# adelacvg/detail_tts

Hardware: AMD Instinct MI355X
Metric: generated audio seconds/sec (24 kHz), 10 s prompt, batch 8 per GPU (higher is better)
Workload: dtype f32; 1 GPU; configs[2]: 1xMI355X batch-8, 10 s prompts (T_ref=936), 234 codes -> 9.984 s audio per utterance; GPT KV-cache decode + 50-step CFG diffusion + flow-VAE/HiFiGAN vocoder, seed-0 random-init weights; batch_per_gpu=8, codes=234, diffusion_steps=50, parallelism=replica x1

## Files before the change

### detail_tts_amd/csrc/model.h

```cpp
#pragma once
#include <map>
#include <memory>
#include <atomic>
#include <thread>
#include <cstring>
#include <memory>
#include <mutex>
#include <string>
#include <unordered_map>
#include <vector>

#include "attention.h"
#include "attn_probs.h"
#include "common.h"
#include "conv_gemm.h"
#include "conv_x3.h"
#include "diff_loss.h"
#include "diff_schedule.h"
#include "disc.h"
#include "flowvae_fwd.h"
#include "gpt_kernels.h"
#include "ops.h"
#include "uncond_cache.h"
#include "../../include/detail_hip.h"

namespace dtts {

struct PackedConv {
    const float* w = nullptr;
    const float* b = nullptr;
    int Cin = 0, CinP = 0, Cout = 0, CoutP = 0, KW = 1;
    const void* w3 = nullptr;
};

static inline int packed_cout(int cout) { return cout > 64 ? round_up(cout, 128) : (cout > 32 ? 64 : 32); }

static inline int gn_groups(int C) {
    int groups = 32;
    while (C % groups) groups /= 2;
    return groups;
}

struct AttnBlockW {
    const float *gn_g = nullptr, *gn_b = nullptr, *bias_tab = nullptr;
    PackedConv qkv, proj;
    int C = 0, H = 0;
};

struct ResBlockW {
    const float *gn1_g = nullptr, *gn1_b = nullptr, *gn2_g = nullptr, *gn2_b = nullptr;
    PackedConv c1, c2, emb;
    int index = 0;
};

struct DiffLayerW {
    ResBlockW rb;
    AttnBlockW at;
};

struct MelStyleW {
    PackedConv sp0, sp1, t0, t1, qkv, afc, fc;
    int n_mel = 0, hidden = 0, out = 0;
};

struct EncLayerW {
    PackedConv qkv, o, f1, f2;
    const float *ek = nullptr, *ev = nullptr, *g1 = nullptr, *b1 = nullptr, *g2 = nullptr, *b2 = nullptr;
};

struct WnW {
    PackedConv cond;
    std::vector<PackedConv> in, res, skip;
    int n_layers = 0;
};

struct CouplingW {
    PackedConv pre, post;
    WnW enc;
};

struct PosteriorW {
    PackedConv pre, proj;
    WnW enc;
    int spec_channels = 0;
};

struct DiscPeriodW {
    const float *w0 = nullptr, *b0 = nullptr;
    PackedConv c[4], post;
};

struct DiscW {
    const float *sw[5] = {nullptr, nullptr, nullptr, nullptr, nullptr}, *sb[5] = {nullptr, nullptr, nullptr, nullptr, nullptr};
    PackedConv s5, s_post;
    DiscPeriodW per[5];
};

struct DiscLayout {
    long long off[DISC_MAPS + 1];
// ... 220 lines not shown
    void op_resblock1(int stage, int branch, const float* x, const int* lens_host, int B, int T, float* y, hipStream_t s);
    void op_wn(int flow, const float* h, const float* g, const int* lens_host, int B, int T, float* out, hipStream_t s);
    void posterior_encode(const float* spec, int spec_ch, const int* lens_host, const float* g, int B, int T, const float* noise, unsigned long long seed,
                          const int* sample_ids_host, float* z, float* m_q, float* logs_q, hipStream_t s);
    void flow_forward(const float* z, const float* g, const int* lens_host, int B, int T, float* z_p, hipStream_t s);
    void slice_segments(const float* x, const int* ids_host, int B, int C, int T, int seg, float* out, hipStream_t s);
    void kl_loss(const float* z_p, const float* logs_q, const float* m_p, const float* logs_p, const int* lens_host, int B, int C, int T,
                 float* out, hipStream_t s);
    void flowvae_forward(const float* mel, const float* spec, int spec_ch, const int* lens_host, int B, int T, const float* noise, unsigned long long seed,
                         const int* sample_ids_host, const int* ids_slice_host, int seg, float* o, float* z, float* z_p, float* m_p,
                         float* logs_p, float* m_q, float* logs_q, float* quantized, hipStream_t s);
    void bind_discriminator(const void* blob, size_t nbytes, const char* const* names, const unsigned long long* offsets,
                            const unsigned long long* numels, int n, hipStream_t stream);
    void disc_forward(const float* y, const float* y_hat, int B, int t, float* maps, hipStream_t s);
    void disc_losses(int n_maps, const float* const* r, const float* const* g, const long long* map_numel, int n_scores,
                     const float* const* dr, const float* const* dg, const long long* score_numel, float* out, hipStream_t s);
    void spec_to_mel(const float* spec, int B, int spec_ch, int T, float* mel_out, hipStream_t s);
    void op_conv1d_grouped(const float* x, const float* w, const float* bias, int B, int Cin, int Tin, int Cout, int groups, int K, int stride,
                           int pad, float slope, float* y, hipStream_t s);
    void op_period_split(const float* wav, int B, int t, int p, float* out, hipStream_t s);
    void flowvae_stage_losses(const float* mel, const float* spec, int spec_ch, const int* lens_host, int B, int T, const float* noise,
                              unsigned long long seed, const int* sample_ids_host, const int* ids_slice_host, int seg, const float* wav, int L,
                              float* o, float* z, float* z_p, float* m_p, float* logs_p, float* m_q, float* logs_q, float* quantized,
                              float* work, float* losses, hipStream_t s);
    void op_enc_p(const float* mel, const int* lens_host, int B, int T, float* m_p, float* logs_p, hipStream_t s);
    void enc_p_fwd(const float* mel, const int* dl, int B, int T, float* x, float* y, float* qkv, float* att, float* ffn, float* relk, float* ml,
                   float* stats, hipStream_t s, bool padded_batch = false);
    void vq_decode(const int* codes_host, const int* ncodes_host, int nmax, const float* refer, const int* refer_lens_host, int Tr,
                   int B, float* mel_out, hipStream_t s, const float* g_in = nullptr);
    void resample(const float* x, int B, int L, const float* kernel, int orig, int neu, int width, float* y, int Lout, hipStream_t s);
    void mel_spectrogram(const float* wav, const int* lens_host, int B, int L, int n_fft, int hop, float* mel_out, int Tmax, hipStream_t s,
                         float* spec_out = nullptr);
    void vq_encode(const float* mel, const int* lens_host, int B, int T, int* codes_out, float* xvq_out, hipStream_t s);
    void op_attention_block(const char* prefix, const float* x, const int* lens_host, int B, int C, int T, float* y, hipStream_t s);
    void op_resblock(const char* prefix, const float* x, const int* lens_host, int B, int T, int step, float* y, hipStream_t s);
    void op_conv1d(const char* name, const float* x, const int* lens_in_host, int B, int Cin, int Tin, int Cout, int KW, int stride,
                   int dil, int pad, int pro_act, int epi_act, int gate, int phases, const float* res, float* y, int Tout_alloc,
                   hipStream_t s);
    void op_conv1d_x3(const char* name, const float* x, const int* lens_host, int B, int Cin, int T, int Cout, int KW, int epi_act,
                      float out_scale, int gate, const float* badd, const float* res, int p1, int ksplit_max, float* y, ConvX3Launch* chosen,
                      hipStream_t s);
    void op_attention_x3(const char* name, const float* x, const int* lens_host, int B, int Cin, int T, int H, const float* bias_tab, int p1,
                         int out_f32, void* y, void* img_out, ConvX3Launch* conv_chosen, AttnX3Launch* attn_chosen, hipStream_t s);
    void op_attention(const float* qkv, const int* lens_host, int B, int rows, int cs, int T, int H, int D, int q_off, int k_off, int v_off,
                      int head_stride, float scale, const float* bias_tab, int causal, const float* band, int band_w, float* y, float* ml,
                      hipStream_t s);
    void op_attention_rel(const float* qkv, const int* lens_host, int B, int T, int H, int D, const float* ek, const float* ev, int W,
                          float scale, float* y, float* relk, float* ml, hipStream_t s);
    void op_philox_normal(float* out, int n, int B, unsigned long long seed, const int* sample_ids_host, int stage, int step,
                          hipStream_t s);

    void set_option(const std::string& key, int value) {
        if (key == "two_streams") opt_two_streams_ = value != 0;
        else if (key == "conv_x3") {
            DTTS_REQUIRE(value != 0 || !opt_trunk_fp16_, "conv_x3 = 0 (exact fp32 kernels) has no trunk_fp16 mode: set trunk_fp16 = 0 first");
            opt_conv_x3_ = value != 0;
        }
        else if (key == "trunk_fp16") {
            DTTS_REQUIRE(value == 0 || value == 1, "trunk_fp16: 0 or 1");
            DTTS_REQUIRE(value == 0 || use_x3(), "trunk_fp16 = 1 needs the split-precision kernels (conv_x3 = 1): the exact fp32 kernels have no one-product mode");
            opt_trunk_fp16_ = value != 0;
        }
        else if (key == "gpt_graph") opt_gpt_graph_ = value != 0;
        else if (key == "x3_range_check") opt_range_check_ = value != 0;
        else if (key == "gpt_token_kernel") { opt_gpt_token_ = value != 0; if (value != 0) tok_failed_ = false; gpt_drop_graphs(); }
        else if (key == "gpt_fuse_proj") { DTTS_REQUIRE(value == 0 || value == 1, "gpt_fuse_proj: 0 or 1"); opt_gpt_fuse_proj_ = value != 0; gpt_drop_graphs(); }
        else if (key == "gpt_token_exclusive_cu") { opt_tok_exclusive_ = value != 0; gpt_drop_graphs(); }
        else if (key == "gpt_token_min_rows") { DTTS_REQUIRE(value == 1 || value == 4 || value == 8, "gpt_token_min_rows: 1, 4 or 8"); opt_tok_min_rows_ = value; gpt_drop_graphs(); }
        else if (key == "gpt_token_wgs") { DTTS_REQUIRE(value == 128 || value == 64 || value == 32, "gpt_token_wgs: 128, 64 or 32"); opt_tok_wgs_ = value; gpt_drop_graphs(); }
        else if (key == "gpt_token_fault") opt_tok_fault_ = value;
        else if (key == "gpt_token_fault_eos") opt_tok_fault_eos_ = value;
        else if (key == "gpt_prompt_raw") opt_prompt_raw_ = value != 0;
        else if (key == "gpt_beam_skip_reorder") { opt_beam_skip_reorder_ = value != 0; gpt_drop_graphs(); }
        else if (key == "cfg_streams") opt_cfg_streams_ = value < 0 ? 0 : value;
        else if (key == "conv_cols") opt_conv_cols_ = value != 0;
        else if (key == "uncond_cache_mb") set_uncond_cache_mb(value);
        else if (key == "voc_chain_planes") opt_voc_chain_ = value != 0;
        else if (key == "voc_x3") opt_voc_x3_ = value != 0;
        else if (key == "x3_fault") opt_x3_fault_ = value;
        else if (key == "attn_ksplit_cus") set_attn_ksplit_cus(value);
        else if (key == "attn_ksplit") set_attn_ksplit(value);
        else if (key == "ln_reg") set_ln_channels_reg(value != 0);
        else if (key == "conv_small_tiles") set_conv_small_tiles(value);
        else if (key == "conv_stages") set_conv_stages(value);
        else throw Error(-1, "unknown option '" + key + "'");
    }
    int get_option(const std::string& key) const {
        if (key == "conv_x3") return use_x3() ? 1 : 0;
        if (key == "trunk_fp16") return opt_trunk_fp16_ ? 1 : 0;
        if (key == "gpt_fuse_proj") return opt_gpt_fuse_proj_ ? 1 : 0;
        throw Error(-1, "option '" + key + "' cannot be read back");
    }
    std::string last_error;
    dtts_config cfg;
    int device;

private:
    friend struct Stage;
    const float* W(const std::string& name, size_t numel) const;
    const float* Wopt(const std::string& name, size_t numel) const;
    PackedConv conv(const std::string& name, int Cin, int Cout, int KW, bool bias = true, int cout_p = 0) const;
    AttnBlockW attn_block(const std::string& prefix, int C, int H) const;
    ResBlockW res_block(const std::string& prefix, int C, int index) const;
    void resblock1_fwd(const ResBlock1W& rb, const float* x, float* tmp, float* out, int ch, const int* lens, int B, int T, hipStream_t s,
                       void* xs = nullptr);
    bool vocoder_x3() const;
    void wn_fwd(const WnW& c, float* h, const float* g, int gin, float* Gc, float* acts, float* h2, float* skip, const int* dl, int B,
                int T, hipStream_t s);
    WnW wn_w(const std::string& prefix, int n_layers) const;
    void enc_q_fwd(const float* spec, int spec_ch, const float* g, const int* dl, int B, int T, float* stats, hipStream_t s);
    void flow_fwd(const float* z, const float* g, const int* dl, int B, int T, float* z_p, hipStream_t s);
    size_t enc_q_ws_bytes(int B, int T) const;
    size_t flow_ws_bytes(int B, int T) const;
    std::vector<int> stage_lens(const int* lens_host, int B, int T, const char* who) const;
    void build_diffusion(hipStream_t s);
    void build_vocoder(hipStream_t s);
    void build_gpt(hipStream_t s);
    void gpt_head_and_sample(hipStream_t s);
    struct GptForced {
        float* enc = nullptr;
        int L = 0;
        std::vector<int> tl, ml;
    };
    struct GptAttnRequest {
        int mode = 0;
        const int* layers = nullptr;
        int n_layers = 0;
        const float* w = nullptr;
        float* out = nullptr;
        int nq_max = 0, nk_max = 0;
    };
    struct GptAttnCapture {
        GptAttnRequest req;
        const int *q0 = nullptr, *nq = nullptr, *k0 = nullptr, *nk = nullptr;
        const float* w = nullptr;
    };
    GptForced gpt_teacher_forced(const float* refer, const int* refer_lens_host, int Tr, const int* text_host, const int* text_lens_host,
                                 int Lt_max, const int* codes_host, const int* ncodes_host, int n_max, int B, size_t extra_ws_bytes,
                                 hipStream_t s, const float* cond_in = nullptr, const GptAttnRequest* attn = nullptr);
    void score_head(const PackedConv& head, const float* lat, long long lat_bs, int lat_cs, const int* targets_host, const int* ntargets_host,
                    int n_max, int B, float* logprob_out, float* logits_out, hipStream_t s);
    void gpt_step_launches(hipStream_t s);
    hipGraphExec_t gpt_capture(int n);
    void gpt_drop_graphs();
    void build_vq();
    void build_frontend();
    void gpt_prefill_layers(float* x, const int* lens, int B, int L, float* kv_cache, long long kv_layer_stride, long long kv_bs,
                            int kv_cs, hipStream_t s, const GptAttnCapture* capture = nullptr);
    void gpt_capture_probs(const GptAttnCapture& c, int layer, const float* qkv, const int* lens, int B, int L, hipStream_t s);
    MelStyleW mel_style_w(const std::string& prefix, int n_mel, int hidden, int out) const;
    ConvParams cp(const float* x, int cin, float* y, int cout, int B, int T, int Ta, const int* lens) const;
    ConvParams cp(const float* x, int cin, int Tin, int Tin_a, const int* len_in, float* y, int cout, int Nout, int Nout_a, const int* len_out,
                  int B) const;
    static void with_planes(ConvParams& p, const void* xs, int T) { p.x3 = xs; p.x3_tp = x3_tp(T); }
    static void with_res(ConvParams& p, const float* res, long long bs, int cs) { p.res = res; p.res_bs = bs; p.res_cs = cs; }

    const int* upload_ints(const int* host, int n, hipStream_t s);
    void register_cols(const int* lens_dev, const int* lens_host, int nb, int T, hipStream_t s);

    void run_conv(const PackedConv& pc, ConvParams p, hipStream_t s, ConvX3Launch* chosen = nullptr) const;
    struct TrunkIo {
        const int* lens;
        int B, T, Ta;
        hipStream_t s;
        float* ab;
        void* xs = nullptr;
        bool p1 = false;
// ... 231 lines not shown
```

### detail_tts_amd/csrc/model.hip

```cpp
#include "model.h"
#include <algorithm>
#include <cmath>
#include <cstring>

namespace dtts {

static thread_local Arena* t_arena_override = nullptr;
Arena* arena_override() { return t_arena_override; }
ArenaUse::ArenaUse(Arena& a) : prev_(t_arena_override) { t_arena_override = &a; }
ArenaUse::~ArenaUse() { t_arena_override = prev_; }

static thread_local bool t_row_invariant = false;
RowInvariantLaunches::RowInvariantLaunches() : prev_(t_row_invariant) { t_row_invariant = true; }
RowInvariantLaunches::~RowInvariantLaunches() { t_row_invariant = prev_; }
bool RowInvariantLaunches::on() { return t_row_invariant; }

Arena::~Arena() {
    if (base_) (void)hipFree(base_);
}

void Arena::ensure(size_t bytes) {
    if (bytes > cap_) {
        DTTS_CHECK_HIP(hipDeviceSynchronize());
        if (base_) DTTS_CHECK_HIP(hipFree(base_));
// ... 200 lines not shown
    r.gn1_b = W(p + ".in_layers.0.bias", C);
    r.c1 = conv(p + ".in_layers.2", C, C, 1);
    r.emb = conv(p + ".emb_layers.1", C, 2 * C, 1);
    r.gn2_g = W(p + ".out_layers.0.weight", C);
    r.gn2_b = W(p + ".out_layers.0.bias", C);
    r.c2 = conv(p + ".out_layers.3", C, C, 3);
    return r;
}

void Model::bind_weights(const void* blob, size_t nbytes, const char* const* names, const unsigned long long* offsets,
                         const unsigned long long* numels, int n, hipStream_t stream) {
    weights_.clear();
    bound_ = false;
    {
        std::lock_guard<std::mutex> lk(ucache_mu_);
        ++bind_gen_;
        ucache_.invalidate_all();
    }
    for (int i = 0; i < n; ++i) {
        DTTS_REQUIRE((offsets[i] + numels[i]) * sizeof(float) <= nbytes, "weight table entry outside the blob");
        DTTS_REQUIRE(offsets[i] % 4 == 0, "weight offsets must be 16-byte aligned");
        weights_[names[i]] = {static_cast<const float*>(blob) + offsets[i], (size_t)numels[i]};
    }
    if (weights_.count("diffusion.inp_block.wp")) build_diffusion(stream);
    has_vocoder_ = weights_.count("dec.conv_pre.wp") != 0;
    if (has_vocoder_) build_vocoder(stream);
    has_gpt_ = weights_.count("gpt.mel_head.wp") != 0;
    if (has_gpt_) build_gpt(stream);
    has_vq_ = weights_.count("quantizer.table") != 0;
    if (has_vq_) build_vq();
    has_frontend_ = weights_.count("frontend.dft.wp") != 0;
    if (has_frontend_) build_frontend();
    bound_ = true;
}

ConvParams Model::cp(const float* x, int cin, float* y, int cout, int B, int T, int Ta, const int* lens) const {
    return cp(x, cin, T, Ta, lens, y, cout, T, Ta, lens, B);
}

ConvParams Model::cp(const float* x, int cin, int Tin, int Tin_a, const int* len_in, float* y, int cout, int Nout, int Nout_a,
                     const int* len_out, int B) const {
    ConvParams p;
    p.B = B;
    p.Tin = Tin;
    p.Nout = Nout;
    p.len_in = len_in;
    p.len_out = len_out;
    p.x = x;
    p.x_bs = (long long)cin * Tin_a;
    p.x_cs = Tin_a;
    p.y = y;
    p.y_bs = (long long)cout * Nout_a;
    p.y_cs = Nout_a;
    return p;
}

static void attach_cols(ConvParams& p) {
    if (t_col_tables.empty() || !p.len_out || p.len_out != p.len_in || p.Nout != p.Tin || p.stride != 1 || p.phases != 1) return;
    for (const ColTable& e : t_col_tables)
        if (p.len_out >= e.lens && p.len_out + p.B <= e.lens + e.nb && p.Nout == e.T) {
            const int b0 = (int)(p.len_out - e.lens), c0 = e.prefix[b0], c1 = e.prefix[b0 + p.B];
            if (c1 > c0 && c1 - c0 < p.B * cdiv(p.Nout, X3_BN)) {
                p.cols = e.cols + c0;
                p.ncols = c1 - c0;
                p.cols_b0 = b0;
            }
            return;
        }
}

void Model::run_conv(const PackedConv& pc, ConvParams p, hipStream_t s, ConvX3Launch* chosen) const {
    p.w = pc.w;
    if (!p.bias) p.bias = pc.b;
    p.Cin = pc.Cin;
    p.CinP = pc.CinP;
    p.Cout = pc.Cout;
    p.CoutP = pc.CoutP;
    p.KW = pc.KW;
    if (p.x3) {
        DTTS_REQUIRE(pc.w3, "conv has no split-precision weights");
        p.w3 = pc.w3;
        attach_cols(p);
        if (RowInvariantLaunches::on()) p.ksplit_max = 1;
        launch_conv_x3(p, s, chosen);
        return;
    }
    launch_conv_gemm(p, s);
}

void Model::op_conv1d(const char* name, const float* x, const int* lens_in_host, int B, int Cin, int Tin, int Cout, int KW,
                      int stride, int dil, int pad, int pro_act, int epi_act, int gate, int phases, const float* res, float* y,
                      int Tout_alloc, hipStream_t s) {
    DTTS_REQUIRE(!weights_.empty(), "weights not bound");
    const int rows = Cout * (phases > 1 ? phases : 1);
    PackedConv pc = conv(name, Cin, rows, KW, Wopt(std::string(name) + ".bp", (size_t)packed_cout(rows)) != nullptr);
    const int Nout = (Tin + 2 * pad - dil * (KW - 1) - 1) / stride + 1;
    std::vector<int> li(B), lo(B);
    for (int b = 0; b < B; ++b) {
        li[b] = lens_in_host ? lens_in_host[b] : Tin;
        lo[b] = (li[b] + 2 * pad - dil * (KW - 1) - 1) / stride + 1;
    }
    const int* dli = upload_ints(li.data(), B, s);
    const int* dlo = upload_ints(lo.data(), B, s);
    const int cout_real = gate ? Cout / 2 : Cout;
    ConvParams p = cp(x, Cin, Tin, Tin, dli, y, cout_real, Nout, Tout_alloc, dlo, B);
    p.stride = stride;
    p.dil = dil;
    p.pad = pad;
    p.pro_act = pro_act;
    p.pro_slope = 0.1f;
    p.epi_act = epi_act;
    p.epi_slope = 0.1f;
    p.gate = gate;
    p.phases = phases > 1 ? phases : 1;
    if (res) with_res(p, res, p.y_bs, Tout_alloc);
    run_conv(pc, p, s);
}

void Model::op_conv1d_x3(const char* name, const float* x, const int* lens_host, int B, int Cin, int T, int Cout, int KW, int epi_act,
                         float out_scale, int gate, const float* badd, const float* res, int p1, int ksplit_max, float* y,
                         ConvX3Launch* chosen, hipStream_t s) {
    DTTS_REQUIRE(!weights_.empty(), "weights not bound");
    DTTS_REQUIRE(name && x && y, "op_conv1d_x3: null argument");
    DTTS_REQUIRE(B > 0 && B <= 65535 && T > 0 && T <= (1 << 20) && Cin > 0 && Cin <= (1 << 16) && Cout > 0 && Cout <= (1 << 16), "op_conv1d_x3: sizes");
    DTTS_REQUIRE(KW == 1 || KW == 3, "op_conv1d_x3: k = 1 or k = 3 (same padding) only");
    DTTS_REQUIRE(Cin % 16 == 0, "op_conv1d_x3: input channels must be a multiple of 16 (one K-step; the split passes write 8-channel chunks)");
    const int CoutP = packed_cout(Cout);
    DTTS_REQUIRE(CoutP % 128 == 0, "op_conv1d_x3: packed output rows must be a multiple of the 128-row tile (Cout > 64)");
    DTTS_REQUIRE(p1 == 0 || p1 == 1, "op_conv1d_x3: p1 is 0 or 1");
    DTTS_REQUIRE(gate == GATE_NONE || gate == GATE_TANH_SIGMOID, "op_conv1d_x3: gate is none or tanh * sigmoid");
    DTTS_REQUIRE(!p1 || (Cin % 32 == 0 && gate == GATE_NONE), "op_conv1d_x3 one-product mode: input channels a multiple of 32, no gate");
    DTTS_REQUIRE(epi_act == ACT_NONE || epi_act == ACT_SILU || epi_act == ACT_LRELU || epi_act == ACT_TANH, "op_conv1d_x3: epilogue activation");
    DTTS_REQUIRE(ksplit_max >= 0, "op_conv1d_x3: ksplit_max");
    const bool rows16 = (reinterpret_cast<unsigned long long>(y) & 15ull) == 0 && T % 4 == 0;
    if (gate != GATE_NONE) {
        DTTS_REQUIRE(KW == 1 && !res && epi_act == ACT_NONE && out_scale == 1.f && Cout % 2 == 0,
                     "op_conv1d_x3 gated epilogue: 1x1 conv, no residual / activation / scale, an even number of rows");
        DTTS_REQUIRE(rows16, "op_conv1d_x3 gated epilogue: rows of y must be 16-byte aligned (T a multiple of 4)");
    } else {
        DTTS_REQUIRE(!badd, "op_conv1d_x3: badd only with the gate");
    }
    const int nt = cdiv(T, X3_BN);
    DTTS_REQUIRE((long long)(CoutP / 128) * nt * B <= (1 << 22), "op_conv1d_x3: launch too large");
    std::vector<int> l(B);
    for (int b = 0; b < B; ++b) {
        l[b] = lens_host ? lens_host[b] : T;
        DTTS_REQUIRE(l[b] >= 0 && l[b] <= T, "op_conv1d_x3: lengths must lie in [0, T]");
    }
    PackedConv pc = conv(name, Cin, Cout, KW, Wopt(std::string(name) + ".bp", (size_t)CoutP) != nullptr);
    DTTS_REQUIRE(pc.CinP == Cin && pc.CoutP == CoutP, "op_conv1d_x3: packed weight shape");
    const size_t w3_bytes = (size_t)KW * (Cin / 8) * 2 * CoutP * 16;
    ws().ensure(w3_bytes + x3_bytes(B, Cin, T) + 8192);
    void* w3 = ws().raw(w3_bytes);
    void* xs = ws().raw(x3_bytes(B, Cin, T));
    launch_split_weights(pc.w, KW, pc.CinP, pc.CoutP, w3, s);
    pc.w3 = w3;
    const int* dl = upload_ints(l.data(), B, s);
    const long long x_bs = (long long)Cin * T;
    launch_split_planes(x, x_bs, T, nullptr, ACT_NONE, dl, T, B, Cin, xs, s);
    register_cols(dl, l.data(), B, T, s);
    ConvParams p = cp(x, Cin, y, gate != GATE_NONE ? Cout / 2 : Cout, B, T, T, dl);
    p.pad = KW == 3 ? 1 : 0;
    p.epi_act = epi_act;
    p.epi_slope = 0.1f;
    p.out_scale = out_scale;
    p.gate = gate;
// ... 176 lines not shown
```

Baseline: 180.5 audio_s/s.

## Add 16x16x32 MFMA variant of split-precision conv kernel and dispatch to it

Adds a new conv_x3s kernel that computes the split-precision (fp16 planes) conv GEMM with mfma_f32_16x16x32_f16 instead of the 32x32x16 shape. It uses hand-scheduled LDS reads with exec-masked half-wave loads, multi-stage global_load_lds pipelining, and optional k-split reduction. The new kernel is selected by default for eligible convs (k=1 or k=3, no gate/activation epilogue), with fallback to the old kernel otherwise. The aim is higher MFMA throughput and better LDS-read overlap in the vocoder and diffusion convs. In exchange it adds a large, complex inline-asm kernel that could carry correctness or register-pressure risk.

```diff
diff --git a/detail_tts_amd/csrc/conv_x3s.h b/detail_tts_amd/csrc/conv_x3s.h
--- /dev/null
+++ b/detail_tts_amd/csrc/conv_x3s.h
@@ -0,0 +1,12 @@
+#pragma once
+#include "conv_x3.h"
+
+namespace dtts {
+
+constexpr int CONV_X3_SHAPE_DEFAULT = 1;
+void set_conv_x3_shape(int v);
+int conv_x3_shape();
+void set_conv_x3s_stages(int n);
+bool launch_conv_x3s(const ConvParams& p, hipStream_t s, ConvX3Launch* chosen = nullptr);
+
+}
diff --git a/detail_tts_amd/csrc/conv_x3s.hip b/detail_tts_amd/csrc/conv_x3s.hip
--- /dev/null
+++ b/detail_tts_amd/csrc/conv_x3s.hip
@@ -0,0 +1,483 @@
+#include <algorithm>
+#include <atomic>
+#include <cstdio>
+#include <cstdlib>
+#include <type_traits>
+#include <utility>
+
+#include "conv_x3s.h"
+#include "prof.h"
+#include "split3.h"
+
+namespace dtts {
+
+typedef float f32x4 __attribute__((ext_vector_type(4)));
+
+namespace {
+constexpr int NPL = XS_PLANES, NK = 2 * NPL;
+constexpr int BM = 128, BN = X3_BN;
+constexpr int WTILE = NK * BM * 16;
+constexpr int XMAIN = NK * BN * 16;
+constexpr int XBUF = XMAIN + NK * 2 * 16;
+
+template <int OFF> __device__ __forceinline__ void rd(hf8& dst, unsigned addr) { asm volatile("ds_read_b128 %0, %1 offset:%2" : "=v"(dst) : "v"(addr), "n"(OFF)); }
+template <int OFF> __device__ __forceinline__ void rd_lo4(hf8 (&a)[4], unsigned wa) {
+    asm volatile("s_mov_b32 exec_hi, 0\n\t"
+                 "ds_read_b128 %0, %4 offset:%5\n\tds_read_b128 %1, %4 offset:%6\n\tds_read_b128 %2, %4 offset:%7\n\tds_read_b128 %3, %4 offset:%8\n\t"
+                 "s_mov_b64 exec, -1"
+                 : "+v"(a[0]), "+v"(a[1]), "+v"(a[2]), "+v"(a[3]) : "v"(wa), "n"(OFF), "n"(OFF + 256), "n"(OFF + 512), "n"(OFF + 768));
+}
+template <int XOFS, int WOFS> __device__ __forceinline__ void rd_hi10(hf8 (&b)[6], hf8 (&a)[4], unsigned xa, unsigned x5, unsigned wa) {
+    asm volatile("s_mov_b32 exec_lo, 0\n\t"
+                 "ds_read_b128 %0, %10 offset:%13\n\tds_read_b128 %1, %10 offset:%14\n\tds_read_b128 %2, %10 offset:%15\n\tds_read_b128 %3, %10 offset:%16\n\t"
+                 "ds_read_b128 %4, %10 offset:%17\n\tds_read_b128 %5, %11 offset:%13\n\t"
+                 "ds_read_b128 %6, %12 offset:%18\n\tds_read_b128 %7, %12 offset:%19\n\tds_read_b128 %8, %12 offset:%20\n\tds_read_b128 %9, %12 offset:%21\n\t"
+                 "s_mov_b64 exec, -1"
+                 : "+v"(b[0]), "+v"(b[1]), "+v"(b[2]), "+v"(b[3]), "+v"(b[4]), "+v"(b[5]), "+v"(a[0]), "+v"(a[1]), "+v"(a[2]), "+v"(a[3])
+                 : "v"(xa), "v"(x5), "v"(wa), "n"(XOFS), "n"(XOFS + 256), "n"(XOFS + 512), "n"(XOFS + 768), "n"(XOFS + 1024), "n"(WOFS), "n"(WOFS + 256),
+                   "n"(WOFS + 512), "n"(WOFS + 768));
+}
+template <class T> struct ic_value { static constexpr int value = 0; };
+template <int V> struct ic_value<std::integral_constant<int, V>> { static constexpr int value = V; };
+template <int N> __device__ __forceinline__ void wait1(hf8& a) { asm volatile("s_waitcnt lgkmcnt(%1)" : "+v"(a) : "n"(N)); }
+template <int N> __device__ __forceinline__ void wait7(hf8 (&b)[6], hf8& a) {
+    asm volatile("s_waitcnt lgkmcnt(%7)" : "+v"(b[0]), "+v"(b[1]), "+v"(b[2]), "+v"(b[3]), "+v"(b[4]), "+v"(b[5]), "+v"(a) : "n"(N));
+}
+
+template <int... K, class F>
+__device__ __forceinline__ void for_each_step(std::integer_sequence<int, K...>, F&& f) {
+    (f(std::integral_constant<int, K>{}), ...);
+}
+
+template <bool KW3, int NSTG>
+__global__ __launch_bounds__(256, 2) void conv_x3s_kernel(ConvParams p) {
+    constexpr int KW = KW3 ? 3 : 1, D = NSTG - 1;
+    constexpr int CB = 2;
+    auto chunk_of = [](int kind) { return (kind & 1) * NPL + (kind >> 1); };
+    constexpr int XOFF = NSTG * WTILE;
+    extern __shared__ __attribute__((aligned(16))) unsigned char smem[];
+    const int tid = threadIdx.x, lane = tid & 63, wave = __builtin_amdgcn_readfirstlane(tid >> 6);
+    const int l15 = lane & 15, kh = (lane >> 4) & 1, hi2 = lane >> 5;
+    const int mtiles = p.CoutP / BM, ntiles = (p.Nout + BN - 1) / BN;
+    const int Ls = xcd_remap(blockIdx.x, gridDim.x);
+    const int S = p.ksplit, L = Ls / S, z = Ls - L * S;
+    const int mt = L % mtiles;
+    int b = (L / mtiles) / ntiles;
+    int nti = (L / mtiles) - b * ntiles;
+    const int bn = L / mtiles;
+    if (p.cols) {
+        const int pk = __builtin_amdgcn_readfirstlane(p.cols[bn]);
+        b = (pk >> 8) - p.cols_b0;
+        nti = pk & 255;
+    }
+    const int m0 = mt * BM, n0 = nti * BN;
+    const int nvalid = p.len_out ? p.len_out[b] : p.Nout;
+    if (n0 >= nvalid) return;
+    const int C8 = p.Cin >> 3, call = p.Cin >> 4, Tp = p.x3_tp;
+    const int cbeg = (int)((long long)call * z / S), c16n = (int)((long long)call * (z + 1) / S) - cbeg, nks = KW * c16n;
+    const int bin = p.x_bidx ? p.x_bidx[b] : b;
+    const unsigned lane16 = (unsigned)lane * 16u;
+    const unsigned char* wb8 = static_cast<const unsigned char*>(p.w3) + ((long long)m0 + (long long)(CB * cbeg) * NPL * p.CoutP) * 16;
+    const unsigned char* xb8 = static_cast<const unsigned char*>(p.x3) +
+                               ((long long)bin * C8 * NPL * Tp + n0 + (X3_HALO - p.pad) + (long long)(CB * cbeg) * NPL * Tp) * 16;
+    const long long wtapB = (long long)C8 * NPL * p.CoutP * 16;
+    const long long wblkB = (long long)CB * NPL * p.CoutP * 16;
+    const long long xblkB = (long long)CB * NPL * Tp * 16;
+    auto dma = [&](const unsigned char* g, int lds_off) {
+        __builtin_amdgcn_global_load_lds((const __attribute__((address_space(1))) void*)(g + lane16),
+                                         (__attribute__((address_space(3))) void*)(smem + lds_off), 16, 0, 0);
+    };
+    const int wkind = wave;
+    const unsigned char* wq = wb8 + (long long)chunk_of(wkind) * p.CoutP * 16;
+    const int wlds = wkind * (BM * 16);
+    const unsigned char* xq = xb8 + (long long)chunk_of(wkind) * Tp * 16;
+    const int xlds = XOFF + wkind * (BN * 16);
+    long long x3o[3];
+    int x3l[3];
+#pragma unroll
+    for (int t = 0; t < 3; ++t) {
+        const int j = t * 4 + wave, kind = j / 3, cb = j - kind * 3;
+        x3o[t] = ((long long)chunk_of(kind) * Tp + cb * 64) * 16;
+        x3l[t] = XOFF + kind * (BN * 16) + cb * 1024;
+    }
+    const long long halo_lane = (lane < 2 * NK) ? (((long long)chunk_of(lane >> 1) * Tp + BN + (lane & 1)) * 16 - (long long)lane16) : 0;
+    const unsigned char* xblk = xb8;
+    auto issue_w = [&](int i, int stage) { dma(wq + i * 1024, stage * WTILE + wlds + i * 1024); };
+    auto issue_x1 = [&](int i, int stage) { dma(xq + i * 1024, stage * XBUF + xlds + i * 1024); };
+    auto issue_x3 = [&](int t, int stage) { dma(xblk + x3o[t], stage * XBUF + x3l[t]); };
+    auto issue_halo = [&](int stage) {
+        if (lane < 2 * NK)
+            __builtin_amdgcn_global_load_lds((const __attribute__((address_space(1))) void*)(xblk + halo_lane + lane16),
+                                             (__attribute__((address_space(3))) void*)(smem + XOFF + stage * XBUF + XMAIN), 16, 0, 0);
+    };
+    int itap = 0;
+    auto next_w = [&]() {
+        if (!KW3) wq += wblkB;
+        else if (itap < 2) { wq += wtapB; ++itap; }
+        else { wq += wblkB - 2 * wtapB; itap = 0; }
+    };
+
+    const int wm0 = (wave >> 1) * 64, wn0 = (wave & 1) * 96;
+    f32x4 acc[4][6];
+#pragma unroll
+    for (int i = 0; i < 4; ++i)
+#pragma unroll
+        for (int j = 0; j < 6; ++j)
+#pragma unroll
+            for (int r = 0; r < 4; ++r) acc[i][j][r] = 0.f;
+
+#pragma unroll
+    for (int q = 0; q < D; ++q) {
+        if (q < nks) {
+            issue_w(0, q);
+            issue_w(1, q);
+        }
+        next_w();
+        if (!KW3) {
+            if (q < nks) {
+#pragma unroll
+                for (int i = 0; i < 3; ++i) issue_x1(i, q);
+            }
+            xq += xblkB;
+        } else {
+            if (q < c16n) {
+#pragma unroll
+                for (int t = 0; t < 3; ++t) issue_x3(t, q);
+                issue_halo(q);
+            }
+            xblk += xblkB;
+        }
+    }
+    float* bias_s = reinterpret_cast<float*>(smem + XOFF + NSTG * XBUF);
+    if (tid < BM) bias_s[tid] = (p.bias && m0 + tid < p.Cout) ? p.bias[m0 + tid] : 0.f;
+
+    hf8 a2[4], r1[6];
+#pragma unroll
+    for (int i = 0; i < 4; ++i) a2[i] = hf8{0, 0, 0, 0, 0, 0, 0, 0};
+#pragma unroll
+    for (int j = 0; j < 6; ++j) r1[j] = hf8{0, 0, 0, 0, 0, 0, 0, 0};
+    constexpr int PLW = 2 * BM * 16, PLX = 2 * BN * 16;
+    const unsigned a_lane = (unsigned)(kh * (BM * 16) + (wm0 + l15) * 16);
+    const unsigned x_lane = (unsigned)(XOFF + kh * (BN * 16) + (wn0 + l15) * 16);
+    const unsigned wa_h = a_lane + (unsigned)(hi2 * PLW);
+    const unsigned xm[3] = {x_lane, x_lane + (unsigned)(hi2 * PLX), x_lane + (unsigned)((1 - hi2) * PLX)};
+    const int pv[3] = {0, hi2, 1 - hi2};
+    unsigned xh5[3];
+#pragma unroll
+    for (int v = 0; v < 3; ++v) xh5[v] = (unsigned)(XOFF + XMAIN + (pv[v] * 2 + kh) * 32 + (wn0 + 80 + l15 - BN) * 16);
+    auto x5_addr = [&](int v, int tp) {
+        if (!KW3) return xm[v] + 1280u;
+        unsigned h = xh5[v];
+        asm volatile("" : "+v"(h));
+        return wn0 + 80 + l15 + tp >= BN ? h : xm[v] + 1280u;
+    };
+    auto mma = [&](const hf8& a, const hf8 (&bb)[6], int i) {
+#pragma unroll
+        for (int j = 0; j < 6; ++j) acc[i][j] = __builtin_amdgcn_mfma_f32_16x16x32_f16(a, bb[j], acc[i][j], 0, 0, 0);
+    };
+
+    int c16 = 0, tap = 0;
+    int sw = 0, sx = 0;
+    auto kstep = [&](auto stw_, auto stx_, auto tp_, auto par_, bool wlive, bool xlive, bool drain) {
+        constexpr int WI = ic_value<decltype(stw_)>::value * WTILE;
+        constexpr int XI = ic_value<decltype(stx_)>::value * XBUF + ic_value<decltype(tp_)>::value * 16;
+        const int stw = stw_, stx = stx_, tp = tp_;
+        const unsigned wd = (unsigned)((stw - ic_value<decltype(stw_)>::value) * WTILE);
+        const unsigned xd = (unsigned)((stx - ic_value<decltype(stx_)>::value) * XBUF + (tp - ic_value<decltype(tp_)>::value) * 16);
+        if (NSTG == 2 || drain) asm volatile("s_waitcnt vmcnt(0)" ::: "memory");
+        else asm volatile("s_waitcnt vmcnt(%0)" ::"n"((NSTG - 2) * (KW3 ? 3 : 5)) : "memory");
+        __builtin_amdgcn_s_barrier();
+        const int swi = stw + D >= NSTG ? stw + D - NSTG : stw + D, sxi = stx + D >= NSTG ? stx + D - NSTG : stx + D;
+        auto slot = [&](int sl) {
+            __builtin_amdgcn_sched_barrier(0);
+            if (sl < 2) { if (wlive) issue_w(sl, swi); }
+            else if (!KW3) { if (xlive) issue_x1(sl - 2, sxi); }
+            else if (sl == 2) { if (xlive) issue_x3(tp, sxi); }
+            else if (sl == 3 && tp == 2) { if (xlive) issue_halo(sxi); }
+            __builtin_amdgcn_sched_barrier(0);
+        };
+        if (decltype(par_)::value == 0) {
+            hf8 a1[4];
+            const unsigned xh = xm[1] + xd, w0 = a_lane + wd;
+            rd<XI>(r1[0], xh); rd<XI + 256>(r1[1], xh); rd<XI + 512>(r1[2], xh); rd<XI + 768>(r1[3], xh); rd<XI + 1024>(r1[4], xh);
+            rd<XI>(r1[5], x5_addr(1, tp) + xd);
+            rd<WI>(a1[0], w0); rd<WI + 256>(a1[1], w0); rd<WI + 512>(a1[2], w0); rd<WI + 768>(a1[3], w0);
+            rd_lo4<WI + PLW>(a2, w0);
+            wait7<7>(r1, a1[0]); mma(a1[0], r1, 0); slot(0);
+            wait1<6>(a1[1]); mma(a1[1], r1, 1); slot(1);
+            wait1<5>(a1[2]); mma(a1[2], r1, 2); slot(2);
+            wait1<4>(a1[3]); mma(a1[3], r1, 3); slot(3);
+            slot(4);
+        } else {
+            hf8 a3[4], r3[6];
+            rd_hi10<XI, WI>(r1, a2, xm[0] + xd, x5_addr(0, tp) + xd, a_lane + wd);
+            const unsigned xn = xm[2] + xd, wh = wa_h + wd;
+            rd<XI>(r3[0], xn); rd<XI + 256>(r3[1], xn); rd<XI + 512>(r3[2], xn); rd<XI + 768>(r3[3], xn); rd<XI + 1024>(r3[4], xn);
+            rd<XI>(r3[5], x5_addr(2, tp) + xd);
+            rd<WI>(a3[0], wh);
+            wait7<10>(r1, a2[0]); mma(a2[0], r1, 0); rd<WI + 256>(a3[1], wh); slot(0);
+            wait1<10>(a2[1]); mma(a2[1], r1, 1); rd<WI + 512>(a3[2], wh); slot(1);
+            wait1<10>(a2[2]); mma(a2[2], r1, 2); rd<WI + 768>(a3[3], wh); slot(2);
+            wait1<10>(a2[3]); mma(a2[3], r1, 3); slot(3);
+            wait7<3>(r3, a3[0]); mma(a3[0], r3, 0); slot(4);
+            wait1<2>(a3[1]); mma(a3[1], r3, 1);
+            wait1<1>(a3[2]); mma(a3[2], r3, 2);
+            wait1<0>(a3[3]); mma(a3[3], r3, 3);
+        }
+    };
+    auto advance = [&]() {
+        next_w();
+        if (!KW3) xq += xblkB;
+        sw = sw + 1 == NSTG ? 0 : sw + 1;
+        if (++tap == KW) {
+            tap = 0;
+            ++c16;
+            sx = sx + 1 == NSTG ? 0 : sx + 1;
+            if (KW3) xblk += xblkB;
+        }
+    };
+    int ks = 0;
+    if (KW3 && (KW * NSTG) % 2 && !(p.ablate & 512)) {
+        while (c16 + 2 + D <= c16n) {
+            for_each_step(std::make_integer_sequence<int, 2 * KW>{}, [&](auto kc) {
+                constexpr int k = decltype(kc)::value, TAPc = k % KW;
+                kstep(sw, sx, std::integral_constant<int, TAPc>{}, std::integral_constant<int, (k & 1)>{}, true, true, false);
+                if ((TAPc + D) % KW < 2) wq += wtapB;
+                else wq += wblkB - 2 * wtapB;
+                sw = sw + 1 == NSTG ? 0 : sw + 1;
+                if (TAPc == KW - 1) {
+                    ++c16;
+                    sx = sx + 1 == NSTG ? 0 : sx + 1;
+                    xblk += xblkB;
+                }
+            });
+            ks += 2 * KW;
+        }
+        itap = D % KW;
+    } else if (KW3 && !(p.ablate & 512)) {
+        constexpr int PERIOD = KW * NSTG, P2 = PERIOD;
+        const int nper = (c16n - D) / (P2 / KW);
+        for (int q = 0; q < nper; ++q) {
+            for_each_step(std::make_integer_sequence<int, P2>{}, [&](auto kc) {
+                constexpr int k = decltype(kc)::value;
+                constexpr int TAPc = k % KW, SWc = k % NSTG, SXc = (k / KW) % NSTG;
+                kstep(std::integral_constant<int, SWc>{}, std::integral_constant<int, SXc>{}, std::integral_constant<int, TAPc>{},
+                      std::integral_constant<int, (k & 1)>{}, true, true, false);
+                if ((TAPc + D) % KW < 2) wq += wtapB;
+                else wq += wblkB - 2 * wtapB;
+                if (TAPc == KW - 1) xblk += xblkB;
+            });
+        }
+        ks = nper * P2;
+        c16 = ks / KW;
+        itap = D % KW;
+    }
+    auto gstep = [&](auto par) {
+        const bool drain = ks + D > nks || (KW3 && c16 + D >= c16n);
+        const bool wlive = ks + D < nks, xlive = KW3 ? c16 + D < c16n : ks + D < nks;
+        kstep(sw, sx, tap, par, wlive, xlive, drain);
+        advance();
+        ++ks;
+    };
+    while (ks + 1 < nks) {
+        gstep(std::integral_constant<int, 0>{});
+        gstep(std::integral_constant<int, 1>{});
+    }
+    if (ks < nks) gstep(std::integral_constant<int, 0>{});
+    if (nks & 1) {
+        if (hi2) {
+#pragma unroll
+            for (int i = 0; i < 4; ++i) a2[i] = hf8{0, 0, 0, 0, 0, 0, 0, 0};
+        }
+        wait7<0>(r1, a2[0]); wait1<0>(a2[1]); wait1<0>(a2[2]); wait1<0>(a2[3]);
+#pragma unroll
+        for (int i = 0; i < 4; ++i) mma(a2[i], r1, i);
+    }
+    asm volatile("s_waitcnt vmcnt(0)" ::: "memory");
+
+    if (S > 1) {
+        float* slab = p.kpart + ((size_t)L * S) * (96 * 256);
+        float* mine = slab + (size_t)z * (96 * 256) + tid;
+#pragma unroll
+        for (int i = 0; i < 4; ++i)
+#pragma unroll
+            for (int j = 0; j < 6; ++j)
+#pragma unroll
+                for (int r = 0; r < 4; ++r) __hip_atomic_store(mine + ((i * 6 + j) * 4 + r) * 256, acc[i][j][r], __ATOMIC_RELAXED, __HIP_MEMORY_SCOPE_AGENT);
+        asm volatile("s_waitcnt vmcnt(0)" ::: "memory");
+        __syncthreads();
+        int* s_last = reinterpret_cast<int*>(bias_s + BM);
+        if (tid == 0) *s_last = __hip_atomic_fetch_add(p.kcount + L, 1, __ATOMIC_RELAXED, __HIP_MEMORY_SCOPE_AGENT) == S - 1 ? 1 : 0;
+        __syncthreads();
+        if (!*s_last) return;
+        if (tid == 0) __hip_atomic_store(p.kcount + L, 0, __ATOMIC_RELAXED, __HIP_MEMORY_SCOPE_AGENT);
+#pragma unroll
+        for (int i = 0; i < 4; ++i)
+#pragma unroll
+            for (int j = 0; j < 6; ++j)
+#pragma unroll
+                for (int r = 0; r < 4; ++r) acc[i][j][r] = 0.f;
+        for (int zz = 0; zz < S; ++zz) {
+            const float* src = slab + (size_t)zz * (96 * 256) + tid;
+#pragma unroll
+            for (int i = 0; i < 4; ++i)
+#pragma unroll
+                for (int j = 0; j < 6; ++j)
+#pragma unroll
+                    for (int r = 0; r < 4; ++r)
+                        acc[i][j][r] += __hip_atomic_load(src + ((i * 6 + j) * 4 + r) * 256, __ATOMIC_RELAXED, __HIP_MEMORY_SCOPE_AGENT);
+        }
+    }
+
+    float* yb = p.y + (long long)b * p.y_bs;
+    const float* rb = p.res ? p.res + (long long)(p.res_bidx ? p.res_bidx[b] : (p.res_bmod ? b % p.res_bmod : b)) * p.res_bs : nullptr;
+    const int q4 = lane >> 4;
+    if (!p.epi_vec) {
+#pragma unroll
+        for (int i = 0; i < 4; ++i)
+#pragma unroll
+            for (int j = 0; j < 6; ++j) {
+                const int n = n0 + wn0 + j * 16 + l15;
+                if (n >= nvalid) continue;
+                float rv[4];
+#pragma unroll
+                for (int r = 0; r < 4; ++r) {
+                    const int row = m0 + wm0 + i * 16 + 4 * q4 + r;
+                    rv[r] = rb ? rb[(long long)(row < p.Cout ? row : p.Cout - 1) * p.res_cs + n] : 0.f;
+                }
+#pragma unroll
+                for (int r = 0; r < 4; ++r) {
+                    const int row = m0 + wm0 + i * 16 + 4 * q4 + r;
+                    if (row >= p.Cout) continue;
+                    yb[(long long)row * p.y_cs + n] = acc[i][j][r] * XS_ACC_SCALE + bias_s[wm0 + i * 16 + 4 * q4 + r] + p.res_scale * rv[r];
+                }
+            }
+        return;
+    }
+    constexpr int EP_LD = 100;
+    const int ncol0 = n0 + wn0;
+    float4 rva[4][6];
+    auto load_res = [&](int q, float4 (&dst)[6]) {
+#pragma unroll
+        for (int k = 0; k < 6; ++k) {
+            const int idx = lane + 64 * k, rl = idx / 24, c4 = idx - rl * 24, row = m0 + wm0 + q * 16 + rl, n = ncol0 + c4 * 4;
+            dst[k] = (row < p.Cout && n < nvalid) ? *reinterpret_cast<const float4*>(rb + (long long)row * p.res_cs + n)
+                                                  : make_float4(0.f, 0.f, 0.f, 0.f);
+        }
+    };
+    if (rb) {
+#pragma unroll
+        for (int q = 0; q < 4; ++q) load_res(q, rva[q]);
+    }
+    __syncthreads();
+    float* st = reinterpret_cast<float*>(smem) + wave * (16 * EP_LD);
+#pragma unroll
+    for (int q = 0; q < 4; ++q) {
+        const int rowt0 = wm0 + q * 16;
+#pragma unroll
+        for (int j = 0; j < 6; ++j)
+#pragma unroll
+            for (int r = 0; r < 4; ++r) st[(4 * q4 + r) * EP_LD + j * 16 + l15] = acc[q][j][r];
+        asm volatile("s_waitcnt lgkmcnt(0)" ::: "memory");
+        __builtin_amdgcn_wave_barrier();
+#pragma unroll
+        for (int k = 0; k < 6; ++k) {
+            const int idx = lane + 64 * k, rl = idx / 24, c4 = idx - rl * 24, row = m0 + rowt0 + rl, n = ncol0 + c4 * 4;
+            const float4 a4 = *reinterpret_cast<const float4*>(st + rl * EP_LD + c4 * 4);
+            const float bz = bias_s[rowt0 + rl];
+            float o[4] = {a4.x * XS_ACC_SCALE + bz, a4.y * XS_ACC_SCALE + bz, a4.z * XS_ACC_SCALE + bz, a4.w * XS_ACC_SCALE + bz};
+            if (rb) {
+                o[0] += p.res_scale * rva[q][k].x; o[1] += p.res_scale * rva[q][k].y; o[2] += p.res_scale * rva[q][k].z; o[3] += p.res_scale * rva[q][k].w;
+            }
+            if (row < p.Cout && n < nvalid) {
+                float* dst = yb + (long long)row * p.y_cs + n;
+                if (n + 3 < nvalid) *reinterpret_cast<float4*>(dst) = make_float4(o[0], o[1], o[2], o[3]);
+                else
+                    for (int e = 0; e < 4 && n + e < nvalid; ++e) dst[e] = o[e];
+            }
+        }
+        asm volatile("s_waitcnt lgkmcnt(0)" ::: "memory");
+        __builtin_amdgcn_wave_barrier();
+    }
+}
+}
+
+static std::atomic<int> g_shape{-1};
+static std::atomic<int> g_stages{-1};
+static int shape_default() {
+    static const int v = env_int("DTTS_CONV_X3_SHAPE", CONV_X3_SHAPE_DEFAULT) != 0 ? 1 : 0;
+    return v;
+}
+void set_conv_x3_shape(int v) {
+    DTTS_REQUIRE(v <= 1, "conv_x3_shape: 0 (32x32x16), 1 (16x16x32 where it applies), < 0 = back to the initial value");
+    g_shape.store(v < 0 ? -1 : v, std::memory_order_relaxed);
+}
+int conv_x3_shape() {
+    const int v = g_shape.load(std::memory_order_relaxed);
+    return v >= 0 ? v : shape_default();
+}
+void set_conv_x3s_stages(int n) { g_stages.store(n < 0 ? -1 : n, std::memory_order_relaxed); }
+
+bool launch_conv_x3s(const ConvParams& p_in, hipStream_t s, ConvX3Launch* chosen) {
+    ConvParams p = p_in;
+    static const int env_ablate = env_int("DTTS_CONV_ABLATE", 0);
+    static const bool epi_vec_on = env_on("DTTS_X3_EPI_VEC");
+    if (env_ablate || p.ablate || p.p1 || p.gate != GATE_NONE || p.badd || p.qkv_planes || p.epi_act != ACT_NONE || p.out_scale != 1.f) return false;
+    if (!p.y || !(p.KW == 1 || p.KW == 3)) return false;
+    auto al16 = [](const void* q, long long bs, int cs) { return (reinterpret_cast<unsigned long long>(q) & 15ull) == 0 && (bs & 3) == 0 && (cs & 3) == 0; };
+    p.epi_vec = (epi_vec_on && al16(p.y, p.y_bs, p.y_cs) && (!p.res || al16(p.res, p.res_bs, p.res_cs))) ? 1 : 0;
+    DTTS_REQUIRE(p.w3 && p.x3 && p.x3_tp > 0, "conv_x3: operands");
+    DTTS_REQUIRE(p.B > 0 && p.Nout > 0 && p.Cout > 0, "empty conv");
+    DTTS_REQUIRE(p.Cin % 16 == 0 && p.CoutP % BM == 0, "conv_x3: channel padding");
+    DTTS_REQUIRE(p.stride == 1 && p.dil == 1 && p.phases == 1, "conv_x3: unsupported conv form");
+    DTTS_REQUIRE((p.KW == 1 && p.pad == 0) || (p.KW == 3 && p.pad == 1), "conv_x3: k = 1 or k = 3 (same padding) only");
+    DTTS_REQUIRE(round_up(p.Nout, BN) + 2 * X3_HALO <= p.x3_tp, "conv_x3: time padding");
+    const int stg_opt = g_stages.load(std::memory_order_relaxed);
+    static const int stg_env = []() { const int n = (int)env_int("DTTS_CONV_STAGES", 0); return n >= 2 && n <= 4 ? n : 0; }();
+    const int force_stg = stg_opt >= 0 ? stg_opt : stg_env;
+    static const long long max3 = env_int("DTTS_CONV_STAGES3_MAXWG", 600);
+    static const long long max4 = env_int("DTTS_CONV_STAGES4_MAXWG", 128);
+    static const long long max4k3 = env_int("DTTS_CONV_STAGES4_MAXWG_K3", 128);
+    DTTS_REQUIRE(!p.cols || (p.ncols > 0 && p.ncols <= cdiv(p.Nout, BN) * p.B && cdiv(p.Nout, BN) < 256), "conv_x3: column table");
+    const long long ntile = (long long)(p.CoutP / BM) * (p.cols ? p.ncols : cdiv(p.Nout, BN) * p.B);
+    const int S = conv_x3_ksplit(p.CoutP, p.Cin, p.KW, p.Nout, p.B, p.ksplit_max);
+    p.ksplit = S;
+    if (S > 1) x3_split_workspace(s, (size_t)ntile * S, &p.kpart, &p.kcount);
+    const long long nwg = ntile * S;
+    const int nstg = force_stg ? force_stg : (nwg <= (p.KW == 3 ? max4k3 : max4) ? 4 : (nwg <= max3 ? 3 : 2));
+    const size_t lds = (size_t)nstg * (WTILE + XBUF) + BM * sizeof(float) + 16;
+    const int l4 = 4 * (WTILE + XBUF) + BM * (int)sizeof(float) + 16;
+    const dim3 grid((unsigned)nwg);
+    const double cols = (double)p.B * p.Nout;
+    const double flops = 2.0 * p.Cout * p.Cin * p.KW * cols;
+    const double bytes = 4.0 * cols * p.Cin + 4.0 * cols * p.Cout * (p.res ? 2.0 : 1.0) + 4.0 * (double)p.Cout * p.Cin * p.KW;
+    {
+        static const bool by_shape = []() { const char* v = env_str("DTTS_PROF_SHAPES"); return v && v[0] == '1'; }();
+        const char* tag = "conv_x3_kernel<128,192>";
+        if (by_shape) tag = p.KW == 3 ? "conv_x3 k3" : (p.Cout > 1024 ? "conv_x3 k1 M=2304" : (p.res ? "conv_x3 k1 +res" : "conv_x3 k1"));
+        ProfScope ps(tag, flops, bytes, s);
+        if (chosen) {
+            chosen->epi = 0;
+            chosen->kw3 = p.KW == 3 ? 1 : 0;
+            chosen->stages = nstg;
+            chosen->ksplit = S;
+            chosen->p1 = 0;
+            chosen->epi_vec = p.epi_vec;
+            chosen->cols = p.cols ? 1 : 0;
+            chosen->workgroups = (int)nwg;
+        }
+#define LAUNCH_X3S(K3)                                                                                            \
+    do {                                                                                                               \
+        if (nstg == 4) { lds_optin(reinterpret_cast<const void*>(conv_x3s_kernel<K3, 4>), l4); hipLaunchKernelGGL((conv_x3s_kernel<K3, 4>), grid, dim3(256), lds, s, p); } \
+        else if (nstg == 3) { lds_optin(reinterpret_cast<const void*>(conv_x3s_kernel<K3, 3>), l4); hipLaunchKernelGGL((conv_x3s_kernel<K3, 3>), grid, dim3(256), lds, s, p); } \
+        else { lds_optin(reinterpret_cast<const void*>(conv_x3s_kernel<K3, 2>), l4); hipLaunchKernelGGL((conv_x3s_kernel<K3, 2>), grid, dim3(256), lds, s, p); } \
+    } while (0)
+        if (p.KW == 3) LAUNCH_X3S(true);
+        else LAUNCH_X3S(false);
+#undef LAUNCH_X3S
+    }
+    DTTS_CHECK_HIP(hipGetLastError());
+    return true;
+}
+
+}
diff --git a/detail_tts_amd/csrc/model.h b/detail_tts_amd/csrc/model.h
--- a/detail_tts_amd/csrc/model.h
+++ b/detail_tts_amd/csrc/model.h
@@ -15,6 +15,7 @@
 #include "common.h"
 #include "conv_gemm.h"
 #include "conv_x3.h"
+#include "conv_x3s.h"
 #include "diff_loss.h"
 #include "diff_schedule.h"
 #include "disc.h"
@@ -401,7 +402,8 @@
         else if (key == "attn_ksplit") set_attn_ksplit(value);
         else if (key == "ln_reg") set_ln_channels_reg(value != 0);
         else if (key == "conv_small_tiles") set_conv_small_tiles(value);
-        else if (key == "conv_stages") set_conv_stages(value);
+        else if (key == "conv_stages") { set_conv_stages(value); set_conv_x3s_stages(value); }
+        else if (key == "conv_x3_shape") set_conv_x3_shape(value);
         else throw Error(-1, "unknown option '" + key + "'");
     }
     int get_option(const std::string& key) const {
diff --git a/detail_tts_amd/csrc/model.hip b/detail_tts_amd/csrc/model.hip
--- a/detail_tts_amd/csrc/model.hip
+++ b/detail_tts_amd/csrc/model.hip
@@ -306,6 +306,7 @@
         p.w3 = pc.w3;
         attach_cols(p);
         if (RowInvariantLaunches::on()) p.ksplit_max = 1;
+        if (conv_x3_shape() && launch_conv_x3s(p, s, chosen)) return;
         launch_conv_x3(p, s, chosen);
         return;
     }
```

Result: no change. 181.5 audio_s/s (median of 6 runs) (+0.5%).
